# yangzhaojason/DualDiff

Hardware: AMD Instinct MI355X
Metric: denoising-steps/sec, 6-view 224×400 fp16, 50-step DDIM @ 1/2/4/8 MI355X (higher is better)
Workload: dtype fp16; 1 GPU; BASELINE configs[1]: 6-view 224x400 (28x50 latents) multiview UNet + 2 ControlNet branches (ORS panorama + ORS-3D, SFA on), CFG 2.0 -> 12 view-instances/scene, DDIM-50 schedule, random-init weights; scenes_per_gpu=1, parallelism=scene-sharded x1 (no data-path collective), hip_graph=True, streams=3, invariant_conditioning=recomputed every step

## Files before the change

### dualdiff_amd/_native.py

```python
import ctypes
import os

import torch
from ctypes import (POINTER, Structure, c_char_p, c_float, c_int32, c_int64, c_uint32, c_void_p)

from . import _build

DD_F16, DD_BF16, DD_F32 = 0, 1, 2
DD_EPI_NONE, DD_EPI_GEGLU, DD_EPI_SILU = 0, 1, 2


class GemmDesc(Structure):
    _fields_ = [
        ("a", c_void_p), ("a2", c_void_p), ("lda", c_int64), ("lda2", c_int64), ("k1", c_int32),
        ("rows", c_int32), ("n", c_int32), ("k", c_int32),
        ("w", c_void_p), ("bias", c_void_p), ("rowvec", c_void_p),
        ("rows_per_inst", c_int32), ("ld_rowvec", c_int32),
        ("res", c_void_p), ("ldres", c_int64),
        ("out", c_void_p), ("ldc", c_int64),
        ("alpha", c_float), ("accumulate", c_int32), ("epilogue", c_int32),
        ("conv", c_int32), ("hin", c_int32), ("win", c_int32), ("cin", c_int32),
        ("hv", c_int32), ("wv", c_int32), ("hout", c_int32), ("wout", c_int32), ("stride", c_int32),
        ("dtype", c_int32), ("tile", c_int32), ("split_k", c_int32),
        ("ws", c_void_p), ("ws_bytes", c_int64),
# ... 26 lines not shown
        ("points", c_void_p), ("classes", c_void_p), ("masks", c_void_p),
        ("class_tokens", c_void_p), ("null_pos", c_void_p), ("null_class", c_void_p),
        ("pos", c_void_p), ("cat", c_void_p), ("cls_out", c_void_p),
        ("rows", c_int32), ("points_per_box", c_int32), ("num_freqs", c_int32), ("include_input", c_int32),
        ("class_token_dim", c_int32), ("cls_offset", c_int32),
        ("ld_cat", c_int64),
        ("normalize", c_int32), ("points_dtype", c_int32), ("dtype", c_int32), ("n_classes", c_int32),
        ("freqs", c_float * 16), ("xyz_min", c_float * 3), ("xyz_range", c_float * 3),
    ]


class XAttnDesc(Structure):
    _fields_ = [
        ("x", c_void_p), ("ldx", c_int64), ("res", c_void_p), ("ldres", c_int64),
        ("wq", c_void_p), ("wo", c_void_p), ("bo", c_void_p),
        ("k", c_void_p), ("v", c_void_p), ("ldk", c_int64), ("ldv", c_int64),
        ("k_inst_stride", c_int64), ("k_head_stride", c_int64), ("v_inst_stride", c_int64), ("v_head_stride", c_int64),
        ("out", c_void_p), ("ldo", c_int64),
        ("instances", c_int32), ("rows_per_inst", c_int32), ("lk", c_int32),
        ("channels", c_int32), ("heads", c_int32), ("scale", c_float), ("dtype", c_int32),
        ("ln_out", c_void_p), ("ld_ln_out", c_int64), ("ln_gamma", c_void_p), ("ln_beta", c_void_p), ("ln_eps", c_float),
        ("lk_dev", c_void_p),
    ]


class Gemm8Desc(Structure):
    _fields_ = [
        ("a", c_void_p), ("a_scale", c_void_p), ("lda", c_int64),
        ("w", c_void_p), ("w_scale", c_void_p), ("ldw", c_int64),
        ("bias", c_void_p), ("res", c_void_p), ("ldres", c_int64),
        ("out", c_void_p), ("ldc", c_int64),
        ("rows", c_int32), ("n", c_int32), ("k_padded", c_int32), ("dtype", c_int32),
        ("out_headmajor_d", c_int32), ("hm_scaled_planes", c_int32), ("hm_scale", c_float), ("geglu", c_int32),
    ]


SIGNATURES = {
    "dd_abi_version": (c_int32, []),
    "dd_desc_size": (c_int64, [c_int32]),
    "dd_error_string": (c_char_p, [c_int32]),
    "dd_target_arch": (c_char_p, []),
    "dd_gemm": (c_int32, [POINTER(GemmDesc), c_void_p]),
    "dd_gemm_workspace_bytes": (c_int64, [POINTER(GemmDesc)]),
    "dd_gemm_num_tiles": (c_int32, []),
    "dd_gemm_tile_id": (c_int32, [c_int32]),
    "dd_gemm_kernel_name": (c_char_p, [POINTER(GemmDesc)]),
    "dd_gemm_conv_pad": (c_int32, [POINTER(GemmDesc), c_int32, c_void_p]),
    "dd_gemm_conv_pad_workspace_bytes": (c_int64, [POINTER(GemmDesc), c_int32]),
    "dd_gemm_conv_pad_kernel_name": (c_char_p, [POINTER(GemmDesc), c_int32]),
    "dd_groupnorm_nhwc": (c_int32, [c_void_p, c_int32, c_void_p, c_int32, c_void_p, c_void_p, c_void_p,
                                    c_int32, c_int32, c_int32, c_float, c_int32, c_int32,
                                    c_void_p, c_int64, c_void_p]),
    "dd_groupnorm_workspace_bytes": (c_int64, [c_int32, c_int32]),
    "dd_groupnorm_is_fused": (c_int32, [c_int32, c_int32, c_int32]),
    "dd_layernorm": (c_int32, [c_void_p, c_void_p, c_void_p, c_void_p, c_int64, c_int32, c_float,
                               c_int32, c_void_p]),
    "dd_attention": (c_int32, [POINTER(AttnDesc), c_void_p]),
    "dd_attention_kernel_name": (c_char_p, [POINTER(AttnDesc)]),
    "dd_add": (c_int32, [c_void_p, c_void_p, c_void_p, c_void_p, c_int64, c_int32, c_void_p]),
    "dd_scale": (c_int32, [c_void_p, c_void_p, c_float, c_int64, c_int32, c_void_p]),
    "dd_probe_spin": (c_int32, [c_void_p, c_uint32, c_void_p]),
    "dd_groupnorm_splitk": (c_int32, [c_void_p, c_int32, c_void_p, c_void_p, c_int32, c_void_p, c_int64, c_void_p,
                                      c_void_p, c_void_p, c_void_p, c_int32, c_int32, c_int32, c_int32, c_float, c_int32,
                                      c_int32, c_void_p]),
    "dd_xattn320": (c_int32, [POINTER(XAttnDesc), c_void_p]),
    "dd_nchw_to_nhwc_views": (c_int32, [c_void_p, c_void_p, c_int32, c_int32, c_int32, c_int32, c_int32, c_int32, c_int32,
                                        c_void_p]),
    "dd_fourier_embed_strided": (c_int32, [c_void_p, c_void_p, c_int64, c_int32, POINTER(c_float), c_int32, c_int32,
                                           c_int32, c_int32, c_int32, c_int64, c_int64, c_int64, c_int64, c_void_p]),
    "dd_box_tokens": (c_int32, [POINTER(BoxTokensDesc), c_void_p]),
    "dd_ctx_assemble": (c_int32, [c_void_p, c_void_p, c_void_p, c_void_p, c_void_p, c_int32, c_int32, c_int32, c_int32,
                                  c_int32, c_int32, c_int32, c_int32, c_void_p]),
    "dd_gemm8": (c_int32, [POINTER(Gemm8Desc), c_void_p]),
    "dd_rowquant_fp8": (c_int32, [c_void_p, c_void_p, c_void_p, c_void_p, c_void_p, c_int64, c_int32, c_int64, c_float,
                                  c_int32, c_void_p]),
    "dd_xattn_pack_weight": (c_int32, [c_void_p, c_void_p, c_int32, c_void_p]),
    "dd_silu": (c_int32, [c_void_p, c_void_p, c_int64, c_int32, c_void_p]),
    "dd_nchw_to_nhwc": (c_int32, [c_void_p, c_void_p, c_int32, c_int32, c_int32, c_int32, c_int32, c_void_p]),
    "dd_nhwc_to_nchw": (c_int32, [c_void_p, c_void_p, c_int32, c_int32, c_int32, c_int32, c_int32, c_void_p]),
    "dd_timestep_embedding": (c_int32, [c_void_p, c_void_p, c_int32, c_int32, c_int32, c_float,
                                        c_int32, c_void_p]),
    "dd_cfg_unipc_step": (c_int32, [c_void_p, c_void_p, c_void_p, c_void_p, c_void_p, c_void_p, c_void_p, c_void_p,
# ... 76 lines not shown
```

### dualdiff_amd/csrc/elementwise.hip

```cpp
#include "dd_common.h"

namespace {

template <typename T>
__global__ __launch_bounds__(256)
void dd_add_kernel(const T* a, const T* b, const T* c, T* y, int64_t nvec) {
  for (int64_t i = (int64_t)blockIdx.x * blockDim.x + threadIdx.x; i < nvec;
       i += (int64_t)gridDim.x * blockDim.x) {
    float fa[8], fb[8];
    dd_unpack8<T>(dd_ld16(a + i * 8), fa);
    dd_unpack8<T>(dd_ld16(b + i * 8), fb);
#pragma unroll
    for (int e = 0; e < 8; ++e) fa[e] += fb[e];
    if (c) {
      dd_unpack8<T>(dd_ld16(c + i * 8), fb);
#pragma unroll
      for (int e = 0; e < 8; ++e) fa[e] += fb[e];
    }
    dd_st16(y + i * 8, dd_pack8<T>(fa));
  }
}

template <typename T, int OP>
__global__ __launch_bounds__(256)
void dd_unary_kernel(const T* x, T* y, float s, int64_t nvec) {
  for (int64_t i = (int64_t)blockIdx.x * blockDim.x + threadIdx.x; i < nvec;
       i += (int64_t)gridDim.x * blockDim.x) {
    float f[8];
    dd_unpack8<T>(dd_ld16(x + i * 8), f);
#pragma unroll
    for (int e = 0; e < 8; ++e) f[e] = OP == 0 ? f[e] * s : dd_silu_f(f[e]);
// ... 393 lines not shown
  if (b < 1) b = 1;
  return (unsigned)b;
}

}

extern "C" int dd_add(const void* a, const void* b, const void* c, void* y, int64_t n,
                      int32_t dtype, dd_stream_t stream) {
  if (!a || !b || !y || n <= 0 || (n & 7)) return DD_ERR_BAD_ARG;
  if (dtype != DD_F16 && dtype != DD_BF16) return DD_ERR_BAD_ARG;
  if (!dd_aligned16(a) || !dd_aligned16(b) || !dd_aligned16(y) || (c && !dd_aligned16(c))) return DD_ERR_BAD_ARG;
  hipStream_t s = reinterpret_cast<hipStream_t>(stream);
  dd_clear_error();
  const int64_t nvec = n / 8;
  if (dtype == DD_F16)
    hipLaunchKernelGGL(dd_add_kernel<_Float16>, dim3(grid_for(nvec)), dim3(256), 0, s,
                       (const _Float16*)a, (const _Float16*)b, (const _Float16*)c, (_Float16*)y, nvec);
  else
    hipLaunchKernelGGL(dd_add_kernel<__bf16>, dim3(grid_for(nvec)), dim3(256), 0, s,
                       (const __bf16*)a, (const __bf16*)b, (const __bf16*)c, (__bf16*)y, nvec);
  return dd_check_launch();
}

extern "C" int dd_scale(const void* x, void* y, float sc, int64_t n, int32_t dtype, dd_stream_t stream) {
  if (!x || !y || n <= 0 || (n & 7)) return DD_ERR_BAD_ARG;
  if (dtype != DD_F16 && dtype != DD_BF16) return DD_ERR_BAD_ARG;
  if (!dd_aligned16(x) || !dd_aligned16(y)) return DD_ERR_BAD_ARG;
  hipStream_t s = reinterpret_cast<hipStream_t>(stream);
  dd_clear_error();
  const int64_t nvec = n / 8;
  if (dtype == DD_F16)
    hipLaunchKernelGGL((dd_unary_kernel<_Float16, 0>), dim3(grid_for(nvec)), dim3(256), 0, s,
                       (const _Float16*)x, (_Float16*)y, sc, nvec);
  else
    hipLaunchKernelGGL((dd_unary_kernel<__bf16, 0>), dim3(grid_for(nvec)), dim3(256), 0, s,
                       (const __bf16*)x, (__bf16*)y, sc, nvec);
  return dd_check_launch();
}

extern "C" int dd_silu(const void* x, void* y, int64_t n, int32_t dtype, dd_stream_t stream) {
  if (!x || !y || n <= 0 || (n & 7)) return DD_ERR_BAD_ARG;
  if (dtype != DD_F16 && dtype != DD_BF16) return DD_ERR_BAD_ARG;
  if (!dd_aligned16(x) || !dd_aligned16(y)) return DD_ERR_BAD_ARG;
  hipStream_t s = reinterpret_cast<hipStream_t>(stream);
  dd_clear_error();
  const int64_t nvec = n / 8;
// ... 343 lines not shown
```

### dualdiff_amd/csrc/norm.hip

```cpp
#include "dd_common.h"
#include <atomic>

namespace {

constexpr int GN_THREADS = 256;
constexpr int GN_MAX_SPLIT = 64;
constexpr int GN_MAX_C = 4096;

struct GnParams {
  const void* x1; const void* x2; int c1, c2, c;
  const void* gamma; const void* beta; void* y;
  int m, hw, groups, cpg; float eps; int silu;
  float* ws;
  int nsplit, pix_per_split;
  const float* sk_part; int sk_nsplit; int64_t sk_rows;
  const void* sk_bias; const void* sk_rowvec; int sk_ld_rowvec;
  const void* sk_res; int64_t sk_ldres;
  void* sk_xout;
};

struct GnMap { int cv_count, pl_count, cv, pl; bool active; };
__device__ __forceinline__ GnMap gn_map(int c) {
  GnMap mp;
  mp.cv_count = c >> 3;
// ... 193 lines not shown
        f[e] = p.silu ? dd_silu_f(y) : y;
      }
      dd_st16(reinterpret_cast<T*>(p.y) + row * p.c + ch, dd_pack8<T>(f));
    };
    int px = p0 + mp.pl;
    if (cv == cv_first && pre_ok) {
#pragma unroll
      for (int u = 0; u < GN_UNROLL; ++u) apply_store(pre[u], (int64_t)inst * p.hw + px + u * mp.pl_count);
      px += GN_UNROLL * mp.pl_count;
    }
    for (; px + (GN_UNROLL - 1) * mp.pl_count < p1; px += GN_UNROLL * mp.pl_count) {
      u32x4 v[GN_UNROLL];
#pragma unroll
      for (int u = 0; u < GN_UNROLL; ++u)
        v[u] = dd_ld16(gn_src<T>(p, (int64_t)inst * p.hw + px + u * mp.pl_count, ch));
#pragma unroll
      for (int u = 0; u < GN_UNROLL; ++u) apply_store(v[u], (int64_t)inst * p.hw + px + u * mp.pl_count);
    }
    for (; px < p1; px += mp.pl_count)
      apply_store(dd_ld16(gn_src<T>(p, (int64_t)inst * p.hw + px, ch)), (int64_t)inst * p.hw + px);
  }
}


template <typename T, int THREADS, int NVMAX, bool SK = false>
__global__ __launch_bounds__(THREADS)
void dd_gn_fused_kernel(const GnParams p, int cpb, int vpp, int plc, int nv, int kred) {
  __shared__ float s_a0[THREADS], s_a1[THREADS], s_q0[THREADS], s_q1[THREADS];
  __shared__ float s_mean[64], s_rstd[64], s_piv[64];
  const int inst = blockIdx.y;
  const int t = threadIdx.x;
  const bool active = t < vpp * plc;
  const int cv = t % vpp, pl = t / vpp;
  const int gpb = cpb / p.cpg;
  const int lch = cv * 8;
  const int g0 = lch / p.cpg;
  const int g1 = min(g0 + 1, gpb - 1);
  const int nfirst = min(8, (g0 + 1) * p.cpg - lch);
  const int ch = blockIdx.x * cpb + min(cv, vpp - 1) * 8;
  u32x4 raw[NVMAX];
#pragma unroll
  for (int i = 0; i < NVMAX; ++i)
    if (i < nv) {
      const int64_t row = (int64_t)inst * p.hw + min(pl + i * plc, p.hw - 1);
      if constexpr (SK) {
        raw[i] = gn_sk_load8<T>(p, row, ch, inst);
// ... 275 lines not shown
  int cpb, vpp, plc, nv, kred, threads;
  if (gn_fused_plan(hw, c, groups, &cpb, &vpp, &plc, &nv, &kred, &threads)) {
    dim3 fgrid(c / cpb, m);
    if (threads == 256) {
      if (dtype == DD_F16) hipLaunchKernelGGL((dd_gn_fused_kernel<_Float16, 256, GNF_NV_SMALL>), fgrid, dim3(256), 0, s, p, cpb, vpp, plc, nv, kred);
      else hipLaunchKernelGGL((dd_gn_fused_kernel<__bf16, 256, GNF_NV_SMALL>), fgrid, dim3(256), 0, s, p, cpb, vpp, plc, nv, kred);
    } else {
      if (dtype == DD_F16) hipLaunchKernelGGL((dd_gn_fused_kernel<_Float16, 1024, GNF_NV_BIG>), fgrid, dim3(1024), 0, s, p, cpb, vpp, plc, nv, kred);
      else hipLaunchKernelGGL((dd_gn_fused_kernel<__bf16, 1024, GNF_NV_BIG>), fgrid, dim3(1024), 0, s, p, cpb, vpp, plc, nv, kred);
    }
    return dd_check_launch();
  }
  dim3 grid(p.nsplit, m);
  if (dtype == DD_F16) {
    hipLaunchKernelGGL(dd_gn_stats_kernel<_Float16>, grid, dim3(GN_THREADS), 0, s, p);
    hipLaunchKernelGGL(dd_gn_apply_kernel<_Float16>, grid, dim3(GN_THREADS), 0, s, p);
  } else {
    hipLaunchKernelGGL(dd_gn_stats_kernel<__bf16>, grid, dim3(GN_THREADS), 0, s, p);
    hipLaunchKernelGGL(dd_gn_apply_kernel<__bf16>, grid, dim3(GN_THREADS), 0, s, p);
  }
  return dd_check_launch();
}

extern "C" int dd_groupnorm_splitk(const float* partial, int32_t nsplit, const void* bias, const void* rowvec,
                                   int32_t ld_rowvec, const void* res, int64_t ldres, void* x_out,
                                   const void* gamma, const void* beta, void* y, int32_t m, int32_t hw, int32_t c,
                                   int32_t groups, float eps, int32_t apply_silu, int32_t dtype, dd_stream_t stream) {
  if (!partial || !gamma || !beta || !y || nsplit < 2 || nsplit > 64) return DD_ERR_BAD_ARG;
  if (m <= 0 || hw <= 0 || groups <= 0 || groups > 64 || c <= 0 || (c & 7) || c % groups || c > GN_MAX_C) return DD_ERR_BAD_ARG;
  if (c / groups < 4) return DD_ERR_UNSUPPORTED;
  if (dtype != DD_F16 && dtype != DD_BF16) return DD_ERR_BAD_ARG;
  if (!dd_aligned16(partial) || !dd_aligned16(y) || !dd_aligned16(gamma) || !dd_aligned16(beta) ||
      (bias && !dd_aligned16(bias)) || (rowvec && (!dd_aligned16(rowvec) || (ld_rowvec & 7))) ||
      (res && (!dd_aligned16(res) || (ldres & 7))) || (x_out && !dd_aligned16(x_out))) return DD_ERR_BAD_ARG;
  int cpb, vpp, plc, nv, kred, threads;
  if (!gn_fused_plan(hw, c, groups, &cpb, &vpp, &plc, &nv, &kred, &threads)) return DD_ERR_UNSUPPORTED;
  GnParams p{};
  p.x1 = nullptr; p.c1 = c; p.c = c;
  p.gamma = gamma; p.beta = beta; p.y = y;
  p.m = m; p.hw = hw; p.groups = groups; p.cpg = c / groups; p.eps = eps; p.silu = apply_silu;
  p.sk_part = partial; p.sk_nsplit = nsplit; p.sk_rows = (int64_t)m * hw;
  p.sk_bias = bias; p.sk_rowvec = rowvec; p.sk_ld_rowvec = ld_rowvec; p.sk_res = res; p.sk_ldres = ldres; p.sk_xout = x_out;
  hipStream_t s = reinterpret_cast<hipStream_t>(stream);
  dd_clear_error();
  dim3 fgrid(c / cpb, m);
  if (threads == 256) {
// ... 40 lines not shown
```

### dualdiff_amd/networks/unet_2d_condition_multiview.py

```python
from dataclasses import dataclass
from typing import Any, Dict, Optional, Tuple, Union

import torch
import torch.nn as nn

from .. import ops as O
from .blocks import BasicMultiviewTransformerBlock
from .layers import (BasicTransformerBlock, prefetch_cross_kv, drop_prefetched_kv, CrossKVBank, Conv3x3, CrossAttnDownBlock2D, CrossAttnUpBlock2D, DownBlock2D, GroupNorm,
                     TimestepEmbedding, Timesteps, UNetMidBlock2DCrossAttn, UpBlock2D, as_nchw_view,
                     run_down_block, run_up_block, to_nhwc, CTX_BASE, context_keys, ctx_capacity, lk_const)
from .model_base import ModelBase, sibling_overlap


def _at_capacity(ctx, cap):
    m, lc, c = ctx.shape
    if lc == cap:
        return ctx
    if ctx.stride(2) == 1 and ctx.stride(1) == c and ctx.stride(0) == cap * c and \
            (ctx.storage_offset() + m * cap * c) * ctx.element_size() <= ctx.untyped_storage().nbytes():
        return ctx.as_strided((m, cap, c), ctx.stride())
    buf = ctx.new_zeros((m, cap, c))
    buf[:, :lc] = ctx
    return buf

# ... 222 lines not shown

    def encode_nhwc(self, x, m, h, w, t_f32, ctx2d, lc):
        dt = self.dtype
        if self.kv_bank:
            if self.__dict__.get("_kv_bank") is None:
                self.__dict__["_kv_bank"] = CrossKVBank(self)
            self.__dict__["_kv_bank"].run(ctx2d)
        elif self.prefetch_kv:
            if self.__dict__.get("_kv_stream") is None:
                self.__dict__["_kv_stream"] = torch.cuda.Stream()
            prefetch_cross_kv(self, ctx2d, self.__dict__["_kv_stream"])
        emb = self.time_embedding.run(self.time_proj.run(t_f32, dt))
        temb = self.temb_bank.run(O.silu(emb))
        forward_size = any(s % (2 ** self.num_upsamplers) != 0 for s in (h, w))
        x = self.conv_in.run(x, m, h, w)
        skips = [(x, h, w)]
        for blk in self.down_blocks:
            x, h, w, s = run_down_block(blk, x, m, h, w, temb, ctx2d, lc)
            skips += s
        x = self.mid_block.run(x, m, h, w, temb, ctx2d, lc)
        return {"x": x, "m": m, "h": h, "w": w, "skips": skips, "temb": temb, "ctx2d": ctx2d, "lc": lc,
                "forward_size": forward_size}

    def decode_nhwc(self, state, down_res=None, mid_res=None):
        x, m, h, w = state["x"], state["m"], state["h"], state["w"]
        skips, temb, ctx2d, lc = list(state["skips"]), state["temb"], state["ctx2d"], state["lc"]

        def plus(t, r):
            if not isinstance(r, (tuple, list)):
                r = (r,)
            if len(r) == 0:
                return t
            i = 0
            while i < len(r):
                t = O.add(t, r[i], r[i + 1]) if i + 1 < len(r) else O.add(t, r[i])
                i += 2
            return t

        if down_res is not None:
            if len(down_res) != len(skips):
                raise ValueError("expected %d down-block residuals, got %d" % (len(skips), len(down_res)))
            skips = [(plus(s, r), sh, sw) for (s, sh, sw), r in zip(skips, down_res)]
        if mid_res is not None:
            x = plus(x, mid_res)
        for i, blk in enumerate(self.up_blocks):
            final = i == len(self.up_blocks) - 1
            k = len(blk.resnets)
            up_size = None
            if not final:
                nxt = skips[-k - 1]
                up_size = (nxt[1], nxt[2]) if state["forward_size"] else None
            x, h, w = run_up_block(blk, x, m, h, w, skips, temb, ctx2d, lc, up_size)
        a = self.conv_norm_out.run(x, m, h * w, True)
        if self.__dict__.get("_kv_stream") is not None:
            drop_prefetched_kv(self, self.__dict__["_kv_stream"])
        if self.__dict__.get("_kv_bank") is not None:
            self.__dict__["_kv_bank"].drop()
        return O.conv3x3_small_cout(a, self.conv_out.packed, self.conv_out.bias, m, h, w)



class UNet2DConditionModel(UNet2DConditionModelMultiview):
    multiview = False



class UNet2DConditionModelMultiviewVideo(UNet2DConditionModelMultiview):
    video = True

    def set_n_frames(self, n_frames):
        from .video_blocks import VideoMultiviewTransformerBlock
        for mod in self.modules():
            if isinstance(mod, VideoMultiviewTransformerBlock):
                mod.n_frames = int(n_frames)
        self.config["n_frames"] = int(n_frames)

    def set_frame_shard(self, shard):
        from .video_blocks import VideoMultiviewTransformerBlock
        blocks = [mod for mod in self.modules() if isinstance(mod, VideoMultiviewTransformerBlock)]
        if shard is not None and any(b.n_frames != shard.plan.n_frames for b in blocks):
            raise ValueError("frame shard plans %d frames, the model is configured for %d"
# ... 5 lines not shown
```

### dualdiff_amd/ops.py

```python
import collections as _collections
import ctypes
import threading as _threading

import torch

from . import _native
from ._native import DD_BF16, DD_EPI_GEGLU, DD_EPI_NONE, DD_EPI_SILU, DD_F16, AttnDesc, Gemm8Desc, GemmDesc, XAttnDesc

_WS = {}
_WS_MIN_BYTES = 64 << 20


class KernelTimer:

    def __init__(self, shapes=False):
        self.records = []
        self.shapes = shapes
        self.overhead_ms = 0.0
        self.empty_bracket_ms = 0.0
        self.probe_ms = 0.0

    def calibrate(self, n=48, probe_us=15.0):
        lib = _native.load()
        st = torch.cuda.current_stream()
# ... 854 lines not shown
        _TIMER.stop(e0, "dd_xattn320_kernel", 4.0 * rows * 320 * 320 + 4.0 * rows * lk * 320,
                    2.0 * (rows * 320 * (2 + (1 if res is not None else 0) + (1 if second is not None else 0))
                           + 2 * 320 * 320 + 2 * instances * lk * 320))
    if second is not None:
        out._ln_out = second
    return out


def add(a, b, c=None, out=None):
    lib = _native.load()
    _need_gpu(a, b, c, out)
    if out is None:
        out = torch.empty_like(a)
    else:
        _forget_derived(out)
    e0 = _TIMER.start() if _TIMER is not None else None
    rc = lib.dd_add(_ptr(a), _ptr(b), _ptr(c), _ptr(out), a.numel(), _dt(a), _stream())
    _native.check(rc, "add")
    if e0 is not None:
        _TIMER.stop(e0, "dd_add", 0.0, 2.0 * a.numel() * (3 + (1 if c is not None else 0)))
    return out


def scale(x, s, out=None):
    lib = _native.load()
    _need_gpu(x, out)
    if out is None:
        out = torch.empty_like(x)
    _native.check(lib.dd_scale(_ptr(x), _ptr(out), s, x.numel(), _dt(x), _stream()), "scale")
    return out


def silu(x, out=None):
    lib = _native.load()
    _need_gpu(x, out)
    if out is None:
        out = torch.empty_like(x)
    _native.check(lib.dd_silu(_ptr(x), _ptr(out), x.numel(), _dt(x), _stream()), "silu")
    return out


def nchw_to_nhwc(x, c_pad=None, views=1):
    lib = _native.load()
    _need_gpu(x)
    m, c, h, wt = x.shape
    if wt % views:
# ... 25 lines not shown
    lib = _native.load()
    _need_gpu(t, out)
    if t.dtype != torch.float32:
        raise TypeError("timesteps must be fp32")
    n = t.numel()
    if out is None:
        out = torch.empty((n, dim), dtype=dtype, device=t.device)
    rc = lib.dd_timestep_embedding(_ptr(t), _ptr(out), n, dim, int(flip_sin_to_cos), freq_shift,
                                   _dt(out), _stream())
    _native.check(rc, "timestep_embedding")
    return out


def conv3x3_small_cout(x, w, bias, m, h, wd, out=None):
    lib = _native.load()
    _need_gpu(x, w, bias, out)
    cin = x.shape[1]
    cout = w.shape[0]
    if out is None:
        out = torch.empty((m, cout, h, wd), dtype=x.dtype, device=x.device)
    rc = lib.dd_conv3x3_small_cout(_ptr(x), _ptr(w), _ptr(bias), _ptr(out), m, h, wd, cin, cout,
                                   _dt(x), _stream())
    _native.check(rc, "conv3x3_small_cout")
    return out


class GivenViews(_collections.namedtuple("GivenViews", "mask clean noise0 gcoef mode")):
    """Given-view state of the fused sampler step (pipeline_bev_controlnet_given_view.py; include/dualdiff_hip.h):
    mask   uint8 device (views,), non-zero for a given view-instance (the latents are `views` equal blocks);
    clean  fp32 device (n...), the clean latents of the given views (any values elsewhere);
    noise0 device (n...) in the latents' dtype, the latents at loop entry;
    gcoef  fp32 device [3], the current row of schedulers.given_view_table (refreshed between graph replays);
    mode   1: re-noise the given views every step (conditional_latents_change_every_input=True), 2: fixed noise."""


def _given_args(g, x):
    _need_gpu(g.mask, g.clean, g.noise0, g.gcoef)
    if g.mode not in (1, 2):
        raise ValueError("given-view mode is 1 (change every input) or 2 (fixed noise), got %r" % (g.mode,))
    if g.mask.dtype != torch.uint8 or g.mask.dim() != 1 or not g.mask.is_contiguous() or g.mask.numel() == 0:
        raise ValueError("given-view mask must be a contiguous uint8 vector with one byte per view-instance")
    if x.numel() % g.mask.numel():
        raise ValueError("%d latent elements are not %d equal views" % (x.numel(), g.mask.numel()))
    if g.clean.dtype != torch.float32 or g.clean.numel() != x.numel() or not g.clean.is_contiguous():
        raise ValueError("given-view clean latents must be contiguous fp32 with the latents' %d elements" % x.numel())
    if g.noise0.dtype != x.dtype or g.noise0.numel() != x.numel() or not g.noise0.is_contiguous():
# ... 286 lines not shown
```

### dualdiff_amd/pipeline/pipeline_bev_controlnet.py

```python
import math
from typing import List, Optional

import torch

from .. import ops as O
from .schedulers import given_view_table, unipc_schedule


def ddim_schedule(num_inference_steps, num_train_timesteps=1000, beta_start=0.00085, beta_end=0.012,
                  steps_offset=1, set_alpha_to_one=False):
    betas = torch.linspace(beta_start ** 0.5, beta_end ** 0.5, num_train_timesteps, dtype=torch.float64) ** 2
    acp = torch.cumprod(1.0 - betas, dim=0)
    ratio = num_train_timesteps // num_inference_steps
    ts = (torch.arange(0, num_inference_steps) * ratio).flip(0) + steps_offset
    coefs = []
    for t in ts.tolist():
        a_t = acp[t]
        prev = t - ratio
        a_p = acp[prev] if prev >= 0 else (torch.tensor(1.0, dtype=torch.float64) if set_alpha_to_one else acp[0])
        coefs.append([a_t.sqrt(), (1 - a_t).sqrt(), a_p.sqrt(), (1 - a_p).sqrt()])
    return ts, torch.tensor(coefs, dtype=torch.float32)


def given_view_inputs(conditional_latents, shape, mask=None, device=None):
# ... 201 lines not shown

            for i in range(1, n):
                run_branch(i)
            if self._prepared is not None:
                tok0 = self._prepared[0]
            else:
                tok0 = self.controlnets[0].prepare_tokens(self.camera_param, self.bboxes_list[0],
                                                          self.prompt_embeds, self.use_aug_text)
            run_branch(0, tok0)
            prep0 = tok0
            if self._segmented:
                for s in self._side:
                    main.wait_stream(s)
            state = self.unet.encode_nhwc(x8, m, h, w, self.t_dev, prep0["ctx2d"], prep0["lc"])
            if not self._segmented:
                for s in self._side:
                    main.wait_stream(s)
            if n == 1:
                down = [r[0] for r in results[0][:-1]]
                mid = results[0][-1][0]
            else:
                down = [tuple(results[i][j][0] for i in range(n)) for j in range(len(results[0]) - 1)]
                mid = tuple(results[i][-1][0] for i in range(n))
            eps = self.unet.decode_nhwc(state, down, mid)
        if self.cfg_half is not None:
            self._eps_half = eps
            return eps
        self._scheduler_step(eps)
        return eps

    def _scheduler_step(self, eps2):
        if self.sampler == "ddim":
            O.cfg_ddim_step(eps2, self.lat2[0], self.coef, self.guidance_scale,
                            x_out=self.lat2[0], x_dup=self.lat2[1], given=self._given)
        else:
            O.cfg_unipc_step(eps2, self.lat2[0], self.hist, self.coef, self.guidance_scale,
                             x_out=self.lat2[0], x_dup=self.lat2[1], given=self._given)

    def _combine_halves(self):
        self._scheduler_step(self.cfg_exchange(self._eps_half))

    def capture(self):
        saved = self.lat2.clone()
        saved_hist = None if self.hist is None else self.hist.clone()

        def restore():
            self.lat2.copy_(saved)
# ... 58 lines not shown
```

### include/dualdiff_hip.h

```cpp
#ifndef DUALDIFF_HIP_H
#define DUALDIFF_HIP_H

#include <stdint.h>

#ifdef __cplusplus
extern "C" {
#endif

#define DD_ABI_VERSION 4

enum { DD_F16 = 0, DD_BF16 = 1 };

enum {
  DD_OK = 0,
  DD_ERR_BAD_ARG = -1,
  DD_ERR_UNSUPPORTED = -2,
  DD_ERR_LAUNCH = -3,
  DD_ERR_WORKSPACE = -4
};

typedef void* dd_stream_t;

int dd_abi_version(void);
int64_t dd_desc_size(int which);
// ... 89 lines not shown
const char* dd_attention_kernel_name(const dd_attn_desc* d);

typedef struct dd_xattn_desc {
  const void* x; int64_t ldx;
  const void* res; int64_t ldres;
  const void* wq; const void* wo; const void* bo;
  const void* k; const void* v; int64_t ldk, ldv;
  int64_t k_inst_stride, k_head_stride, v_inst_stride, v_head_stride;
  void* out; int64_t ldo;
  int32_t instances, rows_per_inst, lk;
  int32_t channels, heads;
  float scale;
  int32_t dtype;
  void* ln_out; int64_t ld_ln_out;
  const void* ln_gamma; const void* ln_beta; float ln_eps;
  const int32_t* lk_dev;
} dd_xattn_desc;

int dd_xattn320(const dd_xattn_desc* d, dd_stream_t stream);
int dd_xattn_pack_weight(const void* w, void* packed, int32_t dtype, dd_stream_t stream);

int dd_add(const void* a, const void* b, const void* c, void* y, int64_t n,
           int32_t dtype, dd_stream_t stream);
int dd_scale(const void* x, void* y, float s, int64_t n, int32_t dtype, dd_stream_t stream);
int dd_silu(const void* x, void* y, int64_t n, int32_t dtype, dd_stream_t stream);

int dd_nchw_to_nhwc(const void* x, void* y, int32_t m, int32_t c, int32_t hw,
                    int32_t c_pad, int32_t dtype, dd_stream_t stream);
int dd_nhwc_to_nchw(const void* x, void* y, int32_t m, int32_t c, int32_t hw,
                    int32_t ldx, int32_t dtype, dd_stream_t stream);

int dd_timestep_embedding(const float* t, void* out, int32_t n, int32_t dim,
                          int32_t flip_sin_to_cos, float freq_shift,
                          int32_t dtype, dd_stream_t stream);

#define DD_F32 2
int dd_fourier_embed(const void* x, void* out, int64_t rows, int32_t dims, const float* freqs,
                     int32_t num_freqs, int32_t include_input, int32_t in_dtype, int32_t out_dtype,
                     dd_stream_t stream);

int dd_nchw_to_nhwc_views(const void* x, void* y, int32_t m, int32_t c, int32_t h, int32_t w, int32_t views,
                          int32_t c_pad, int32_t dtype, dd_stream_t stream);
int dd_fourier_embed_strided(const void* x, void* out, int64_t rows, int32_t dims, const float* freqs,
                             int32_t num_freqs, int32_t include_input, int32_t in_dtype, int32_t out_dtype,
                             int32_t inner, int64_t stride_outer, int64_t stride_inner, int64_t stride_dim,
                             int64_t out_ld, dd_stream_t stream);
// ... 3 lines not shown
  void* pos; void* cat; void* cls_out;
  int32_t rows, points_per_box, num_freqs, include_input, class_token_dim, cls_offset;
  int64_t ld_cat;
  int32_t normalize, points_dtype, dtype;
  int32_t n_classes;
  float freqs[16]; float xyz_min[3]; float xyz_range[3];
} dd_box_tokens_desc;
int dd_box_tokens(const dd_box_tokens_desc* d, dd_stream_t stream);
int dd_ctx_assemble(const void* cam, const void* text, const void* box, void* full, void* txt, int32_t m,
                    int32_t n_cam, int32_t lt, int32_t nbox, int32_t dim, int32_t text_per_view, int32_t box_views,
                    int32_t dtype, dd_stream_t stream);

int dd_ors_project(const uint8_t* occ, const float* origin, const float* dir, uint8_t* labels, void* cond,
                   int32_t n_cam, int32_t hw, int32_t samples, float step, int32_t keep_fg, int32_t keep_bg,
                   int32_t dtype, dd_stream_t stream);

int dd_softmax_rows(const float* s, void* p, int64_t rows, int32_t cols, int64_t lds, int64_t ldp,
                    int32_t dtype, dd_stream_t stream);

int dd_conv3x3_small_cout(const void* x, const void* w, const void* bias, void* y_nchw,
                          int32_t m, int32_t h, int32_t wd, int32_t cin, int32_t cout,
                          int32_t dtype, dd_stream_t stream);

int dd_vae_posterior(const void* moments, const float* wq, const float* bq, const void* noise, void* z,
                     int32_t m, int32_t h, int32_t w, float scale, int32_t out_f32, int32_t dtype, dd_stream_t stream);

int dd_clip_embed(const int64_t* ids, const void* tok, const void* pos, void* out, int32_t* pool_index,
                  int32_t batch, int32_t l, int32_t c, int32_t vocab, int32_t eos_token_id, int32_t dtype,
                  dd_stream_t stream);

#define DD_CAUSAL_ATTN_MAX_L 128
int dd_causal_attention(const void* q, const void* k, const void* v, void* o, int64_t ldq, int64_t ldk, int64_t ldv,
                        int64_t ldo, int64_t q_batch_stride, int64_t k_batch_stride, int64_t v_batch_stride,
                        int64_t o_batch_stride, int32_t batch, int32_t l, int32_t heads, int32_t head_dim, float scale,
                        int32_t dtype, dd_stream_t stream);

int dd_conv3x3_thin(const void* x, const void* w, const void* bias, void* y, int32_t m, int32_t hin, int32_t win,
                    int32_t cin, int32_t cout, int32_t stride, int32_t silu, int32_t dtype, dd_stream_t stream);

int dd_cfg_ddim_step(const void* eps, const void* x, void* x_out, void* x_dup,
                     const float* coef, float guidance, int64_t n,
                     int32_t dtype, dd_stream_t stream);

int dd_cfg_unipc_step(const void* eps, const void* x, void* x_out, void* x_dup, float* last, float* m1,
                      float* m2, const float* coef, float guidance, int64_t n, int32_t dtype,
                      dd_stream_t stream);
// ... 37 lines not shown
```

Baseline: 91.40 steps/s.

## Batch ControlNet residual adds into one launch and fuse GroupNorm+SiLU into conv_out

```diff
diff --git a/dualdiff_amd/_native.py b/dualdiff_amd/_native.py
--- a/dualdiff_amd/_native.py
+++ b/dualdiff_amd/_native.py
@@ -72,6 +72,10 @@
         ("ln_out", c_void_p), ("ld_ln_out", c_int64), ("ln_gamma", c_void_p), ("ln_beta", c_void_p), ("ln_eps", c_float),
         ("lk_dev", c_void_p),
     ]
+
+
+class AddEntry(Structure):
+    _fields_ = [("a", c_void_p), ("b", c_void_p), ("c", c_void_p), ("y", c_void_p), ("n", c_int64)]
 
 
 class Gemm8Desc(Structure):
@@ -108,6 +112,10 @@
     "dd_attention": (c_int32, [POINTER(AttnDesc), c_void_p]),
     "dd_attention_kernel_name": (c_char_p, [POINTER(AttnDesc)]),
     "dd_add": (c_int32, [c_void_p, c_void_p, c_void_p, c_void_p, c_int64, c_int32, c_void_p]),
+    "dd_add_multi": (c_int32, [POINTER(AddEntry), c_int32, c_int32, c_void_p]),
+    "dd_gn_conv_out": (c_int32, [c_void_p, c_void_p, c_void_p, c_void_p, c_void_p, c_void_p, c_int32, c_int32, c_int32,
+                                 c_int32, c_int32, c_int32, c_float, c_int32, c_int32, c_void_p, c_int64, c_void_p]),
+    "dd_gn_conv_out_supported": (c_int32, [c_int32, c_int32, c_int32, c_int32, c_int32]),
     "dd_scale": (c_int32, [c_void_p, c_void_p, c_float, c_int64, c_int32, c_void_p]),
     "dd_probe_spin": (c_int32, [c_void_p, c_uint32, c_void_p]),
     "dd_groupnorm_splitk": (c_int32, [c_void_p, c_int32, c_void_p, c_void_p, c_int32, c_void_p, c_int64, c_void_p,
diff --git a/dualdiff_amd/csrc/elementwise.hip b/dualdiff_amd/csrc/elementwise.hip
--- a/dualdiff_amd/csrc/elementwise.hip
+++ b/dualdiff_amd/csrc/elementwise.hip
@@ -7,6 +7,46 @@
 void dd_add_kernel(const T* a, const T* b, const T* c, T* y, int64_t nvec) {
   for (int64_t i = (int64_t)blockIdx.x * blockDim.x + threadIdx.x; i < nvec;
        i += (int64_t)gridDim.x * blockDim.x) {
+    float fa[8], fb[8];
+    dd_unpack8<T>(dd_ld16(a + i * 8), fa);
+    dd_unpack8<T>(dd_ld16(b + i * 8), fb);
+#pragma unroll
+    for (int e = 0; e < 8; ++e) fa[e] += fb[e];
+    if (c) {
+      dd_unpack8<T>(dd_ld16(c + i * 8), fb);
+#pragma unroll
+      for (int e = 0; e < 8; ++e) fa[e] += fb[e];
+    }
+    dd_st16(y + i * 8, dd_pack8<T>(fa));
+  }
+}
+
+struct dd_add_multi_args {
+  const void* a[DD_ADD_MULTI_MAX]; const void* b[DD_ADD_MULTI_MAX]; const void* c[DD_ADD_MULTI_MAX];
+  void* y[DD_ADD_MULTI_MAX]; int64_t nvec[DD_ADD_MULTI_MAX]; uint32_t blk_end[DD_ADD_MULTI_MAX];
+};
+
+template <typename T>
+__global__ __launch_bounds__(256)
+void dd_add_multi_kernel(const dd_add_multi_args args) {
+  const uint32_t blk = blockIdx.x;
+  const void *pa = args.a[0], *pb = args.b[0], *pc = args.c[0];
+  void* py = args.y[0];
+  int64_t nvec = args.nvec[0];
+  uint32_t first = 0, end = args.blk_end[0];
+#pragma unroll
+  for (int e = 1; e < DD_ADD_MULTI_MAX; ++e) {
+    if (blk >= args.blk_end[e - 1]) {
+      pa = args.a[e]; pb = args.b[e]; pc = args.c[e]; py = args.y[e]; nvec = args.nvec[e];
+      first = args.blk_end[e - 1]; end = args.blk_end[e];
+    }
+  }
+  const T* a = reinterpret_cast<const T*>(pa);
+  const T* b = reinterpret_cast<const T*>(pb);
+  const T* c = reinterpret_cast<const T*>(pc);
+  T* y = reinterpret_cast<T*>(py);
+  const int64_t stride = (int64_t)(end - first) * 256;
+  for (int64_t i = (int64_t)(blk - first) * 256 + threadIdx.x; i < nvec; i += stride) {
     float fa[8], fb[8];
     dd_unpack8<T>(dd_ld16(a + i * 8), fa);
     dd_unpack8<T>(dd_ld16(b + i * 8), fb);
@@ -446,6 +486,27 @@
   return dd_check_launch();
 }
 
+extern "C" int dd_add_multi(const dd_add_entry* entries, int32_t count, int32_t dtype, dd_stream_t stream) {
+  if (!entries || count <= 0 || count > DD_ADD_MULTI_MAX) return DD_ERR_BAD_ARG;
+  if (dtype != DD_F16 && dtype != DD_BF16) return DD_ERR_BAD_ARG;
+  dd_add_multi_args args{};
+  uint32_t blocks = 0;
+  for (int e = 0; e < count; ++e) {
+    const dd_add_entry& d = entries[e];
+    if (!d.a || !d.b || !d.y || d.n <= 0 || (d.n & 7)) return DD_ERR_BAD_ARG;
+    if (!dd_aligned16(d.a) || !dd_aligned16(d.b) || !dd_aligned16(d.y) || (d.c && !dd_aligned16(d.c))) return DD_ERR_BAD_ARG;
+    args.a[e] = d.a; args.b[e] = d.b; args.c[e] = d.c; args.y[e] = d.y; args.nvec[e] = d.n / 8;
+    blocks += grid_for(d.n / 8);
+    args.blk_end[e] = blocks;
+  }
+  for (int e = count; e < DD_ADD_MULTI_MAX; ++e) args.blk_end[e] = blocks;
+  hipStream_t s = reinterpret_cast<hipStream_t>(stream);
+  dd_clear_error();
+  if (dtype == DD_F16) hipLaunchKernelGGL(dd_add_multi_kernel<_Float16>, dim3(blocks), dim3(256), 0, s, args);
+  else hipLaunchKernelGGL(dd_add_multi_kernel<__bf16>, dim3(blocks), dim3(256), 0, s, args);
+  return dd_check_launch();
+}
+
 extern "C" int dd_scale(const void* x, void* y, float sc, int64_t n, int32_t dtype, dd_stream_t stream) {
   if (!x || !y || n <= 0 || (n & 7)) return DD_ERR_BAD_ARG;
   if (dtype != DD_F16 && dtype != DD_BF16) return DD_ERR_BAD_ARG;
diff --git a/dualdiff_amd/csrc/norm.hip b/dualdiff_amd/csrc/norm.hip
--- a/dualdiff_amd/csrc/norm.hip
+++ b/dualdiff_amd/csrc/norm.hip
@@ -239,6 +239,184 @@
   }
 }
 
+
+constexpr int GCO_THREADS = 512, GCO_PIX = 96, GCO_SEG = GCO_PIX / 16;
+constexpr int GCO_LDS_LIMIT = 160 * 1024 - 4096;
+
+__host__ __device__ inline int gco_pitch(int c) { return c * 2 + 16; }
+__host__ __device__ inline int gco_staged(int wd) { return GCO_PIX + 2 * wd + 2; }
+
+template <typename T, int NCH2>
+__global__ __launch_bounds__(GCO_THREADS)
+void dd_gn_conv_out_kernel(const GnParams p, const T* __restrict__ w, const T* __restrict__ bias, T* __restrict__ y,
+                           int h, int wd, int cout) {
+  using V8 = typename dd_vec<T>::v8;
+  extern __shared__ __attribute__((aligned(16))) unsigned char gco_smem[];
+  __shared__ float s_mean[64], s_rstd[64];
+  __shared__ float s_ps[GN_THREADS], s_pq[GN_THREADS];
+  const int tid = threadIdx.x, lane = tid & 63, wave = tid >> 6;
+  const int px = lane & 15, kc = lane >> 4;
+  const int sg = wave & 3, kh = wave >> 2;
+  const int inst = blockIdx.y, hw = p.hw, c = p.c;
+  const int p0 = blockIdx.x * GCO_PIX;
+  const int pitch = gco_pitch(c), npix = gco_staged(wd);
+  const int q0 = p0 - wd - 1;
+  f32x4* red = reinterpret_cast<f32x4*>(gco_smem + (size_t)npix * pitch);
+
+  V8 wf[9][NCH2];
+#pragma unroll
+  for (int tap = 0; tap < 9; ++tap)
+#pragma unroll
+    for (int i = 0; i < NCH2; ++i) {
+      u32x4 val = {0u, 0u, 0u, 0u};
+      if (px < cout) val = dd_ld16(w + ((int64_t)px * 9 + tap) * c + (kh * NCH2 + i) * 32 + kc * 8);
+      wf[tap][i] = dd_as_v8<T>(val);
+    }
+
+  const float my_pivot = tid < p.groups ? gn_pivot<T>(p, inst, tid) : 0.f;
+  if (tid < GN_THREADS) {
+    const int g = tid % p.groups;
+    const int chunk = tid / p.groups;
+    const int nchunk = GN_THREADS / p.groups;
+    float s = 0.f, ss = 0.f;
+    if (chunk < nchunk) {
+      const float* src = p.ws + ((int64_t)inst * p.nsplit * p.groups + g) * 2;
+      for (int i = chunk; i < p.nsplit; i += nchunk) {
+        s += src[(int64_t)i * p.groups * 2];
+        ss += src[(int64_t)i * p.groups * 2 + 1];
+      }
+    }
+    s_ps[tid] = s;
+    s_pq[tid] = ss;
+  }
+  __syncthreads();
+  if (tid < p.groups) {
+    const int nchunk = GN_THREADS / p.groups;
+    float a = 0.f, b = 0.f;
+    for (int k = 0; k < nchunk; ++k) { a += s_ps[k * p.groups + tid]; b += s_pq[k * p.groups + tid]; }
+    const float inv_n = 1.0f / ((float)p.hw * (float)p.cpg);
+    const float dm = a * inv_n;
+    const float var = fmaxf(b * inv_n - dm * dm, 0.f);
+    s_mean[tid] = my_pivot + dm;
+    s_rstd[tid] = rsqrtf(var + p.eps);
+  }
+  __syncthreads();
+
+  {
+    const int cvc = c >> 3;
+    const int plc = GCO_THREADS / cvc;
+    const int cv = tid % cvc, pl = tid / cvc;
+    if (pl < plc) {
+      const int ch = cv << 3;
+      float ga[8], be[8], sc[8], sh[8];
+      dd_unpack8<T>(dd_ld16(reinterpret_cast<const T*>(p.gamma) + ch), ga);
+      dd_unpack8<T>(dd_ld16(reinterpret_cast<const T*>(p.beta) + ch), be);
+#pragma unroll
+      for (int e = 0; e < 8; ++e) {
+        const int g = (ch + e) / p.cpg;
+        sc[e] = s_rstd[g] * ga[e];
+        sh[e] = be[e] - s_mean[g] * sc[e];
+      }
+      const T* xin = reinterpret_cast<const T*>(p.x1) + (int64_t)inst * hw * c + ch;
+      unsigned char* dst = gco_smem + cv * 16;
+      for (int s0 = pl; s0 < npix; s0 += GN_UNROLL * plc) {
+        u32x4 v[GN_UNROLL];
+        bool in[GN_UNROLL];
+#pragma unroll
+        for (int u = 0; u < GN_UNROLL; ++u) {
+          const int q = q0 + s0 + u * plc;
+          in[u] = s0 + u * plc < npix && q >= 0 && q < hw;
+          v[u] = u32x4{0u, 0u, 0u, 0u};
+          if (in[u]) v[u] = dd_ld16(xin + (int64_t)q * c);
+        }
+#pragma unroll
+        for (int u = 0; u < GN_UNROLL; ++u) {
+          const int sl = s0 + u * plc;
+          if (sl >= npix) break;
+          if (in[u]) {
+            float f[8];
+            dd_unpack8<T>(v[u], f);
+#pragma unroll
+            for (int e = 0; e < 8; ++e) {
+              const float yv = f[e] * sc[e] + sh[e];
+              f[e] = p.silu ? dd_silu_f(yv) : yv;
+            }
+            v[u] = dd_pack8<T>(f);
+          }
+          *reinterpret_cast<u32x4*>(dst + (size_t)sl * pitch) = v[u];
+        }
+      }
+    }
+  }
+  __syncthreads();
+
+  f32x4 acc[2];
+#pragma unroll
+  for (int r = 0; r < 2; ++r) {
+    const int seg = sg + 4 * r;
+    acc[r] = f32x4{0.f, 0.f, 0.f, 0.f};
+    if (seg >= GCO_SEG || p0 + seg * 16 >= hw) continue;
+    const int pp = p0 + seg * 16 + px;
+    const int oy = pp / wd, ox = pp - oy * wd;
+    const unsigned char* base = gco_smem + (size_t)(seg * 16 + px) * pitch + (kh * NCH2 * 32 + kc * 8) * 2;
+#pragma unroll
+    for (int tap = 0; tap < 9; ++tap) {
+      const int ky = tap / 3, kx = tap - ky * 3;
+      const bool ok = pp < hw && (unsigned)(oy + ky - 1) < (unsigned)h && (unsigned)(ox + kx - 1) < (unsigned)wd;
+      const unsigned char* src = base + (size_t)(ky * wd + kx) * pitch;
+#pragma unroll
+      for (int i = 0; i < NCH2; ++i) {
+        u32x4 xv = *reinterpret_cast<const u32x4*>(src + i * 64);
+        if (!ok) xv = u32x4{0u, 0u, 0u, 0u};
+        acc[r] = dd_mfma16(wf[tap][i], dd_as_v8<T>(xv), acc[r]);
+      }
+    }
+    if (kh == 1) red[seg * 64 + lane] = acc[r];
+  }
+  __syncthreads();
+  if (kh == 0) {
+#pragma unroll
+    for (int r = 0; r < 2; ++r) {
+      const int seg = sg + 4 * r;
+      const int pp = p0 + seg * 16 + px;
+      if (seg >= GCO_SEG || pp >= hw) continue;
+      const f32x4 hi = red[seg * 64 + lane];
+#pragma unroll
+      for (int e = 0; e < 4; ++e) {
+        const int o = kc * 4 + e;
+        if (o < cout) {
+          const float bv = bias ? (float)bias[o] : 0.f;
+          y[((int64_t)inst * cout + o) * hw + pp] = (T)(acc[r][e] + hi[e] + bv);
+        }
+      }
+    }
+  }
+}
+
+inline size_t gco_lds_bytes(int wd, int c) {
+  return (size_t)gco_staged(wd) * gco_pitch(c) + (size_t)GCO_SEG * 64 * sizeof(f32x4);
+}
+
+template <typename T, int NCH2>
+void gco_launch(const GnParams& p, const void* w, const void* bias, void* y, int h, int wd, int cout, hipStream_t s) {
+  const size_t smem = gco_lds_bytes(wd, p.c);
+  auto kern = dd_gn_conv_out_kernel<T, NCH2>;
+  static std::atomic<uint64_t> attr_done{0};
+  dd_ensure_dyn_lds(reinterpret_cast<const void*>(kern), smem, attr_done);
+  hipLaunchKernelGGL(kern, dim3((p.hw + GCO_PIX - 1) / GCO_PIX, p.m), dim3(GCO_THREADS), smem, s, p,
+                     (const T*)w, (const T*)bias, (T*)y, h, wd, cout);
+}
+
+template <typename T>
+void gco_launch_t(const GnParams& p, const void* w, const void* bias, void* y, int h, int wd, int cout, hipStream_t s) {
+  switch (p.c / 64) {
+    case 1: gco_launch<T, 1>(p, w, bias, y, h, wd, cout, s); break;
+    case 2: gco_launch<T, 2>(p, w, bias, y, h, wd, cout, s); break;
+    case 3: gco_launch<T, 3>(p, w, bias, y, h, wd, cout, s); break;
+    case 4: gco_launch<T, 4>(p, w, bias, y, h, wd, cout, s); break;
+    default: gco_launch<T, 5>(p, w, bias, y, h, wd, cout, s); break;
+  }
+}
 
 template <typename T, int THREADS, int NVMAX, bool SK = false>
 __global__ __launch_bounds__(THREADS)
@@ -560,6 +738,43 @@
   return dd_check_launch();
 }
 
+extern "C" int dd_gn_conv_out_supported(int32_t h, int32_t wd, int32_t cin, int32_t cout, int32_t groups) {
+  if (h <= 0 || wd <= 0 || cin <= 0 || cout <= 0 || groups <= 0) return 0;
+  if ((cin & 63) || cin > 320 || cout > 8 || groups > 64 || cin % groups || cin / groups < 4) return 0;
+  if ((int64_t)h * wd > INT32_MAX / 2) return 0;
+  return gco_lds_bytes(wd, cin) <= (size_t)GCO_LDS_LIMIT ? 1 : 0;
+}
+
+extern "C" int dd_gn_conv_out(const void* x, const void* gamma, const void* beta, const void* w, const void* bias,
+                              void* y_nchw, int32_t m, int32_t h, int32_t wd, int32_t cin, int32_t cout, int32_t groups,
+                              float eps, int32_t apply_silu, int32_t dtype, void* ws, int64_t ws_bytes,
+                              dd_stream_t stream) {
+  if (!x || !gamma || !beta || !w || !y_nchw || !ws) return DD_ERR_BAD_ARG;
+  if (m <= 0 || h <= 0 || wd <= 0 || cin <= 0 || cout <= 0 || groups <= 0) return DD_ERR_BAD_ARG;
+  if (dtype != DD_F16 && dtype != DD_BF16) return DD_ERR_BAD_ARG;
+  if (!dd_aligned16(x) || !dd_aligned16(gamma) || !dd_aligned16(beta) || !dd_aligned16(w) ||
+      (reinterpret_cast<uintptr_t>(bias) & 1u) || (reinterpret_cast<uintptr_t>(y_nchw) & 1u)) return DD_ERR_BAD_ARG;
+  if (!dd_gn_conv_out_supported(h, wd, cin, cout, groups) || m > 65535) return DD_ERR_UNSUPPORTED;
+  if (ws_bytes < dd_groupnorm_workspace_bytes(m, groups)) return DD_ERR_WORKSPACE;
+  GnParams p{};
+  p.x1 = x; p.c1 = cin; p.c = cin;
+  p.gamma = gamma; p.beta = beta;
+  p.m = m; p.hw = h * wd; p.groups = groups; p.cpg = cin / groups; p.eps = eps; p.silu = apply_silu;
+  p.ws = reinterpret_cast<float*>(ws) + 64;
+  p.nsplit = gn_plan(p.hw, cin, &p.pix_per_split);
+  hipStream_t s = reinterpret_cast<hipStream_t>(stream);
+  dd_clear_error();
+  dim3 grid(p.nsplit, m);
+  if (dtype == DD_F16) {
+    hipLaunchKernelGGL(dd_gn_stats_kernel<_Float16>, grid, dim3(GN_THREADS), 0, s, p);
+    gco_launch_t<_Float16>(p, w, bias, y_nchw, h, wd, cout, s);
+  } else {
+    hipLaunchKernelGGL(dd_gn_stats_kernel<__bf16>, grid, dim3(GN_THREADS), 0, s, p);
+    gco_launch_t<__bf16>(p, w, bias, y_nchw, h, wd, cout, s);
+  }
+  return dd_check_launch();
+}
+
 extern "C" int dd_groupnorm_splitk(const float* partial, int32_t nsplit, const void* bias, const void* rowvec,
                                    int32_t ld_rowvec, const void* res, int64_t ldres, void* x_out,
                                    const void* gamma, const void* beta, void* y, int32_t m, int32_t hw, int32_t c,
diff --git a/dualdiff_amd/networks/unet_2d_condition_multiview.py b/dualdiff_amd/networks/unet_2d_condition_multiview.py
--- a/dualdiff_amd/networks/unet_2d_condition_multiview.py
+++ b/dualdiff_amd/networks/unet_2d_condition_multiview.py
@@ -268,7 +268,8 @@
         return {"x": x, "m": m, "h": h, "w": w, "skips": skips, "temb": temb, "ctx2d": ctx2d, "lc": lc,
                 "forward_size": forward_size}
 
-    def decode_nhwc(self, state, down_res=None, mid_res=None):
+    def decode_nhwc(self, state, down_res=None, mid_res=None, side_stream=None):
+        env = __import__('os').environ
         x, m, h, w = state["x"], state["m"], state["h"], state["w"]
         skips, temb, ctx2d, lc = list(state["skips"]), state["temb"], state["ctx2d"], state["lc"]
 
@@ -283,13 +284,51 @@
                 i += 2
             return t
 
-        if down_res is not None:
-            if len(down_res) != len(skips):
-                raise ValueError("expected %d down-block residuals, got %d" % (len(skips), len(down_res)))
-            skips = [(plus(s, r), sh, sw) for (s, sh, sw), r in zip(skips, down_res)]
-        if mid_res is not None:
-            x = plus(x, mid_res)
+        def as_tuple(r):
+            return tuple(r) if isinstance(r, (tuple, list)) else (r,)
+
+        if down_res is not None and len(down_res) != len(skips):
+            raise ValueError("expected %d down-block residuals, got %d" % (len(skips), len(down_res)))
+        res = [as_tuple(r) for r in (down_res or [()] * len(skips))] + [() if mid_res is None else as_tuple(mid_res)]
+        late_join = None
+        if env.get("DD_ADD_MULTI", "1") != "0" and all(len(r) <= 2 for r in res):
+            n_first = len(self.up_blocks) // 2
+            cut = len(skips) - sum(len(b.resnets) for b in self.up_blocks[:n_first])
+            tens = [s[0] for s in skips] + [x]
+            first = [i for i in range(cut, len(tens)) if res[i]]
+            late = [i for i in range(cut) if res[i]]
+            if len(first) > O.ADD_MULTI_MAX or len(late) > O.ADD_MULTI_MAX:
+                raise NotImplementedError("more than %d residual sums per decoder half" % O.ADD_MULTI_MAX)
+
+            def launch(idx, outs=None):
+                ents = [(tens[i], res[i][0], res[i][1] if len(res[i]) > 1 else None) +
+                        (() if outs is None else (outs[k],)) for k, i in enumerate(idx)]
+                for i, t in zip(idx, O.add_multi(ents)):
+                    tens[i] = t
+
+            if first:
+                launch(first)
+            if late:
+                if side_stream is not None and env.get("DD_ADD_MULTI_SIDE", "1") != "0":
+                    main = torch.cuda.current_stream()
+                    outs = [torch.empty_like(tens[i]) for i in late]
+                    side_stream.wait_stream(main)
+                    with torch.cuda.stream(side_stream):
+                        launch(late, outs)
+                    late_join = (n_first, side_stream)
+                else:
+                    launch(late)
+            skips = [(t, sh, sw) for t, (_, sh, sw) in zip(tens[:-1], skips)]
+            x = tens[-1]
+        else:
+            if down_res is not None:
+                skips = [(plus(s, r), sh, sw) for (s, sh, sw), r in zip(skips, down_res)]
+            if mid_res is not None:
+                x = plus(x, mid_res)
         for i, blk in enumerate(self.up_blocks):
+            if late_join is not None and i == late_join[0]:
+                torch.cuda.current_stream().wait_stream(late_join[1])
+                late_join = None
             final = i == len(self.up_blocks) - 1
             k = len(blk.resnets)
             up_size = None
@@ -297,12 +336,19 @@
                 nxt = skips[-k - 1]
                 up_size = (nxt[1], nxt[2]) if state["forward_size"] else None
             x, h, w = run_up_block(blk, x, m, h, w, skips, temb, ctx2d, lc, up_size)
-        a = self.conv_norm_out.run(x, m, h * w, True)
+        if late_join is not None:
+            torch.cuda.current_stream().wait_stream(late_join[1])
         if self.__dict__.get("_kv_stream") is not None:
             drop_prefetched_kv(self, self.__dict__["_kv_stream"])
         if self.__dict__.get("_kv_bank") is not None:
             self.__dict__["_kv_bank"].drop()
-        return O.conv3x3_small_cout(a, self.conv_out.packed, self.conv_out.bias, m, h, w)
+        gn, co = self.conv_norm_out, self.conv_out
+        if (env.get("DD_GN_CONV_OUT", "1") != "0" and getattr(x, "_gn_cache", None) is None
+                and not getattr(x, "_unwritten", False)
+                and O.gn_conv_out_ok(h, w, x.shape[1], co.out_channels, gn.num_groups)):
+            return O.gn_conv_out(x, gn.weight, gn.bias, co.packed, co.bias, m, h, w, gn.num_groups, gn.eps, True)
+        a = gn.run(x, m, h * w, True)
+        return O.conv3x3_small_cout(a, co.packed, co.bias, m, h, w)
 
 
 
diff --git a/dualdiff_amd/ops.py b/dualdiff_amd/ops.py
--- a/dualdiff_amd/ops.py
+++ b/dualdiff_amd/ops.py
@@ -900,6 +900,38 @@
     return out
 
 
+ADD_MULTI_MAX = 16
+
+
+def add_multi(entries):
+    lib = _native.load()
+    if not 0 < len(entries) <= ADD_MULTI_MAX:
+        raise ValueError("add_multi takes 1..%d entries, got %d" % (ADD_MULTI_MAX, len(entries)))
+    table = (_native.AddEntry * len(entries))()
+    outs = []
+    dt = _dt(entries[0][0])
+    for d, ent in zip(table, entries):
+        a, b, c = ent[:3]
+        out = ent[3] if len(ent) > 3 else None
+        _need_gpu(a, b, c, out)
+        if _dt(a) != dt or b.dtype != a.dtype or (c is not None and c.dtype != a.dtype):
+            raise TypeError("add_multi: one dtype per launch")
+        if b.numel() != a.numel() or (c is not None and c.numel() != a.numel()):
+            raise ValueError("add_multi: operands of an entry must have the same size")
+        if out is None:
+            out = torch.empty_like(a)
+        else:
+            _forget_derived(out)
+        d.a, d.b, d.c, d.y, d.n = a.data_ptr(), b.data_ptr(), None if c is None else c.data_ptr(), out.data_ptr(), a.numel()
+        outs.append(out)
+    e0 = _TIMER.start() if _TIMER is not None else None
+    _native.check(lib.dd_add_multi(table, len(entries), dt, _stream()), "add_multi")
+    if e0 is not None:
+        _TIMER.stop(e0, "dd_add_multi", 0.0,
+                    sum(2.0 * e[0].numel() * (3 + (1 if e[2] is not None else 0)) for e in entries))
+    return outs
+
+
 def scale(x, s, out=None):
     lib = _native.load()
     _need_gpu(x, out)
@@ -971,6 +1003,29 @@
     rc = lib.dd_conv3x3_small_cout(_ptr(x), _ptr(w), _ptr(bias), _ptr(out), m, h, wd, cin, cout,
                                    _dt(x), _stream())
     _native.check(rc, "conv3x3_small_cout")
+    return out
+
+
+def gn_conv_out_ok(h, wd, cin, cout, groups):
+    return bool(_native.load().dd_gn_conv_out_supported(h, wd, cin, cout, groups))
+
+
+def gn_conv_out(x, gamma, beta, w, bias, m, h, wd, groups, eps, silu=True, out=None):
+    lib = _native.load()
+    _need_gpu(x, gamma, beta, w, bias, out)
+    if not x.is_contiguous():
+        raise ValueError("gn_conv_out input must be contiguous")
+    cin, cout = x.shape[1], w.shape[0]
+    if out is None:
+        out = torch.empty((m, cout, h, wd), dtype=x.dtype, device=x.device)
+    ws = workspace(lib.dd_groupnorm_workspace_bytes(m, groups), x.device, "gn")
+    e0 = _TIMER.start() if _TIMER is not None else None
+    rc = lib.dd_gn_conv_out(_ptr(x), _ptr(gamma), _ptr(beta), _ptr(w), _ptr(bias), _ptr(out), m, h, wd, cin, cout,
+                            groups, eps, int(silu), _dt(x), _ptr(ws), ws.numel() * 4, _stream())
+    _native.check(rc, "gn_conv_out")
+    if e0 is not None:
+        _TIMER.stop(e0, "dd_gn_stats_kernel + dd_gn_conv_out_kernel (2 launches)", 2.0 * 9 * cin * cout * m * h * wd,
+                    4.0 * x.numel())
     return out
 
 
diff --git a/dualdiff_amd/pipeline/pipeline_bev_controlnet.py b/dualdiff_amd/pipeline/pipeline_bev_controlnet.py
--- a/dualdiff_amd/pipeline/pipeline_bev_controlnet.py
+++ b/dualdiff_amd/pipeline/pipeline_bev_controlnet.py
@@ -247,7 +247,7 @@
             else:
                 down = [tuple(results[i][j][0] for i in range(n)) for j in range(len(results[0]) - 1)]
                 mid = tuple(results[i][-1][0] for i in range(n))
-            eps = self.unet.decode_nhwc(state, down, mid)
+            eps = self.unet.decode_nhwc(state, down, mid, side_stream=None if self._segmented else self._side[0])
         if self.cfg_half is not None:
             self._eps_half = eps
             return eps
diff --git a/include/dualdiff_hip.h b/include/dualdiff_hip.h
--- a/include/dualdiff_hip.h
+++ b/include/dualdiff_hip.h
@@ -135,6 +135,11 @@
 
 int dd_add(const void* a, const void* b, const void* c, void* y, int64_t n,
            int32_t dtype, dd_stream_t stream);
+#define DD_ADD_MULTI_MAX 16
+typedef struct {
+  const void* a; const void* b; const void* c; void* y; int64_t n;
+} dd_add_entry;
+int dd_add_multi(const dd_add_entry* entries, int32_t count, int32_t dtype, dd_stream_t stream);
 int dd_scale(const void* x, void* y, float s, int64_t n, int32_t dtype, dd_stream_t stream);
 int dd_silu(const void* x, void* y, int64_t n, int32_t dtype, dd_stream_t stream);
 
@@ -184,6 +189,11 @@
                           int32_t m, int32_t h, int32_t wd, int32_t cin, int32_t cout,
                           int32_t dtype, dd_stream_t stream);
 
+int dd_gn_conv_out(const void* x, const void* gamma, const void* beta, const void* w, const void* bias, void* y_nchw,
+                   int32_t m, int32_t h, int32_t wd, int32_t cin, int32_t cout, int32_t groups, float eps,
+                   int32_t apply_silu, int32_t dtype, void* ws, int64_t ws_bytes, dd_stream_t stream);
+int dd_gn_conv_out_supported(int32_t h, int32_t wd, int32_t cin, int32_t cout, int32_t groups);
+
 int dd_vae_posterior(const void* moments, const float* wq, const float* bq, const void* noise, void* z,
                      int32_t m, int32_t h, int32_t w, float scale, int32_t out_f32, int32_t dtype, dd_stream_t stream);
 
```

Result: no change. 91.87 steps/s (median of 6 runs) (+0.5%).
